# IBM/spark-s3-shuffle

Hardware: AMD Instinct MI355X
Metric: shuffle_block_compress_checksum_throughput (higher is better)
Workload: dtype u8; 1 GPU; terasort-10g-200p-lz4; direction=compress, codec=lz4, checksum=adler32, partitions_per_map_task=200, map_task_bytes=134217700, map_tasks_per_gpu=8, task_threads_per_gpu=4, map_tasks_per_library_call=2, inputs=resident in HBM

## Files before the change

### spark-s3-shuffle_amd/csrc/lz4_window_engine.inc

```

#if defined(S3S_ENGINE_NO_SPEC)
#undef S3S_ENGINE_SPEC
#elif !defined(S3S_ENGINE_SPEC)
#define S3S_ENGINE_SPEC 1
#endif

#if defined(S3S_ENGINE_NO_DEFER) || !defined(S3S_ENGINE_SPEC)
#undef S3S_ENGINE_DEFER
#elif !defined(S3S_ENGINE_DEFER)
#define S3S_ENGINE_DEFER 1
#endif

#ifdef S3S_LZ4_RING
#if !defined(S3S_ENGINE_SPEC) || !defined(S3S_ENGINE_DEFER) || defined(S3S_ENGINE_PW_DIRECT) || defined(S3S_ENGINE_DLOAD_20)
#error "S3S_LZ4_RING is built on the shipped block (speculative gather, deferred emission, 64-lane stream load)"
#endif
#define S3S_RING_SPAN "0xe80"
#define S3S_RING_BYTES 4096
#define S3S_RING_SPAN_N 0xe80
#define S3S_RING_AHEAD 316
#define S3S_RING_LANES 60
#if S3S_RING_SPAN_N - 1 + 64 + S3S_RING_AHEAD > S3S_RING_BYTES || 63 + 4 + 4 * (S3S_RING_LANES - 1) + 8 > S3S_RING_AHEAD
#error "S3S_RING_SPAN / S3S_RING_LANES no longer fit what the ring holds behind and ahead of a window"
#endif
#define S3S_RING_WRITE(OFF)                  \
  "v_add_u32_e32 v158, " OFF ", v158\n\t"                                                                  \
  "v_and_b32_e32 v158, 0xfff, v158\n\t"                                                                    \
  "ds_write_b32 v158, v154 offset:16384\n\t"
#define S3S_RING_FILL_ISSUE       \
  "v_lshl_add_u32 v150, v129, 4, s76\n\t"                                                                  \
  "v_add_u32_e32 v151, 0xfffff040, v150\n\t"                                                               \
  "v_add_u32_e32 v152, 0xfffff440, v150\n\t"                                                               \
  "v_add_u32_e32 v153, 0xfffff840, v150\n\t"                                                               \
// ... 48 lines not shown
  "s_and_saveexec_b64 s[84:85], s[82:83]\n\t"                                                              \
  "v_sub_u32_e32 v123, s97, v129\n\t"                                                                      \
  "v_sub_u32_e32 v124, s98, v129\n\t"                                                                      \
  "v_and_b32_e32 v123, 0xfff, v123\n\t"                                                                    \
  "v_and_b32_e32 v124, 0xfff, v124\n\t"                                                                    \
  "ds_read_u8 v127, v123 offset:16384\n\t"                                                                 \
  "ds_read_u8 v128, v124 offset:16384\n\t"                                                                 \
  "s_mov_b64 exec, s[84:85]\n\t"
#define S3S_RING_EXT(NB)                                                                                      \
  "s_cmpk_lt_u32 s98, " S3S_RING_SPAN "\n\t"                                                               \
  "s_cbranch_scc0 .Lw_extg" NB "_%=\n\t"                                                                   \
  S3S_RING_ISSUE                                                                                           \
  "s_and_b32 s97, s87, 0xc00000\n\t"                                                                       \
  "s_cbranch_scc1 .Lw_mfullr" NB "_%=\n\t"                                                                 \
  ".Lw_fwonlyr" NB "_%=:\n\t"                                                                              \
  S3S_RING_FIN                                                                                             \
  "v_xor_b32_e32 v123, v150, v151\n\t"                                                                     \
  "s_branch .Lw_fwc2" NB "_%=\n\t"                                                                        \
  ".Lw_mfullr" NB "_%=:\n\t"                                                                               \
  "s_bitcmp1_b32 s87, 23\n\t"                                                                              \
  "s_cbranch_scc1 .Lw_extbr" NB "_%=\n\t"                                                                  \
  "s_cmp_gt_i32 s92, 4\n\t"                                                                                \
  "s_cbranch_scc0 .Lw_fwonlyr" NB "_%=\n\t"                                                                \
  ".Lw_extbr" NB "_%=:\n\t"                                                                                \
  S3S_RING_BWD                                                                                             \
  S3S_RING_FIN                                                                                             \
  "v_cmp_ne_u32_e64 s[84:85], v127, v128\n\t"                                                              \
  "v_xor_b32_e32 v123, v150, v151\n\t"                                                                     \
  "s_branch .Lw_extbc2" NB "_%=\n\t"                                                                        \
    \
  ".Lw_mfullx" NB "_%=:\n\t"                                                                               \
  "s_bitcmp1_b32 s87, 23\n\t"                                                                              \
  "s_cbranch_scc1 .Lw_extbx" NB "_%=\n\t"                                                                  \
  "s_cmp_gt_i32 s92, 4\n\t"                                                                                \
  "s_cbranch_scc0 .Lw_exthw" NB "_%=\n\t"                                                                  \
  ".Lw_extbx" NB "_%=:\n\t"                                                                                \
  "s_sub_i32 s98, s89, s88\n\t"                                                                            \
  "s_cmpk_lt_u32 s98, " S3S_RING_SPAN "\n\t"                                                               \
  "s_cbranch_scc0 .Lw_extb" NB "_%=\n\t"                                                                   \
  S3S_RING_BWD                                                                                             \
  "s_waitcnt vmcnt(2) lgkmcnt(0)\n\t"                                                                      \
  "s_branch .Lw_extbc" NB "_%=\n\t"                                                                        \
  ".Lw_extg" NB "_%=:\n\t"
#define S3S_RING_EXTFULL(NB)                                                                                  \
  "s_cmpk_lt_u32 s98, " S3S_RING_SPAN "\n\t"                                                               \
  "s_cbranch_scc0 .Lw_extfg" NB "_%=\n\t"                                                                  \
  S3S_RING_ISSUE                                                                                           \
  "s_branch .Lw_extbr" NB "_%=\n\t"                                                                        \
  ".Lw_extfg" NB "_%=:\n\t"
#define S3S_RING_EXTBC(NB) ".Lw_extbc" NB "_%=:\n\t"
#define S3S_RING_EXTBC2(NB) ".Lw_extbc2" NB "_%=:\n\t"
#define S3S_RING_FWC2(NB) ".Lw_fwc2" NB "_%=:\n\t"
#define S3S_RING_EXTH_MFULL(NB) "s_cbranch_scc1 .Lw_mfullx" NB "_%=\n\t"
#define S3S_RING_EXTHW(NB) ".Lw_exthw" NB "_%=:\n\t"
#else
#define S3S_RING_WRITE(OFF)
#define S3S_RING_FILL_ISSUE
#define S3S_RING_FILL_WRITE
#define S3S_RING_EXT(NB)
#define S3S_RING_EXTFULL(NB)
#define S3S_RING_EXTBC(NB)
#define S3S_RING_EXTBC2(NB)
#define S3S_RING_FWC2(NB)
#define S3S_RING_EXTH_MFULL(NB) "s_cbranch_scc1 .Lw_mfull" NB "_%=\n\t"
#define S3S_RING_EXTHW(NB)
#endif

#ifdef S3S_ENGINE_ABL_NOSTORE
#define S3S_ENGINE_STORE ""
#else
#define S3S_ENGINE_STORE "global_store_byte v124, v122, %[outp]\n\t"
#endif

#ifdef S3S_ABL_CLAMP_FAR
#define S3S_ENGINE_STR_(x) #x
#define S3S_ENGINE_STR(x) S3S_ENGINE_STR_(x)
#define S3S_ENGINE_ABL_CLAMP "v_add_u32_e32 v152, -" S3S_ENGINE_STR(S3S_ABL_CLAMP_FAR) ", v148\n\tv_max_i32_e32 v150, v150, v152\n\t"
#else
#define S3S_ENGINE_ABL_CLAMP ""
#endif
#ifdef S3S_ABL_DUP_PW
#define S3S_ENGINE_ABL_DUP_PW "global_load_dwordx4 v[160:163], v148, %[inp] offset:124\n\t"
#else
// ... 244 lines not shown
  "ds_write_b16 v149, v148\n\t"                                                                            \
  "ds_read_u16 v128, v149\n\t"
#define S3S_SPEC_PASS2_AND_NEXT_GATHER(GN)                                                                    \
  "s_waitcnt lgkmcnt(0)\n\t"                                 \
  "v_cmp_ne_u32_e64 %[Dp], v128, v148\n\t"                                                                 \
  \
  "s_mov_b64 exec, -1\n\t"                                                                                 \
  "v_add_u32_e32 v150, -4, v159\n\t"                                                                       \
  "v_max_i32_e32 v150, 0, v150\n\t"                                                                        \
  "global_load_dwordx4 " GN ", v150, %[inp]" S3S_ENGINE_GATHER_POL "\n\t"                                    \
  "s_mov_b64 exec, %[Dp]\n\t"                                                                              \
  "ds_write_b16 v149, v148\n\t"                                                                            \
  "s_mov_b64 exec, s[74:75]\n\t"                                                                           \
  "ds_read_u16 v128, v149\n\t"  \
  S3S_ENGINE_RUN_INIT
#define S3S_SPEC_PASS2_DONE(FILL)                                                                             \
  "s_waitcnt lgkmcnt(0)\n\t"                                                                               \
  "v_cmp_ne_u32_e64 s[84:85], v128, v148\n\t"                                      \
  FILL                                                                                                     \
  "s_or_b64 %[Dp], %[Dp], s[84:85]\n\t"                                                                    \
  "s_andn2_b64 exec, s[74:75], s[84:85]\n\t"                                                               \
  "ds_write_b16 v149, %[cp]\n\t"                                                                           \
  "s_mov_b64 exec, -1\n\t"
#define S3S_ENGINE_FIXED(NB, Y0, Y1, Y2, Y3, Z0, Z1, Z2, Z3, G, G0, G1, G2, G3, GN)                            \
  ".Lw_winf" NB "_%=:\n\t"                                                                                 \
  S3S_SPEC_HEAD(Z0, Z1, Z2, Z3, "v_cmp_ne_u32_e64 vcc, %[cp], v159\n\t")                     \
  "v_mov_b32_e32 v150, 0x80000000\n\t"  \
  "v_cndmask_b32_e32 %[info], %[info], v150, vcc\n\t"                         \
  "v_cmp_ne_u32_e64 s[82:83], 0, %[info]\n\t"          \
  S3S_SPEC_PASS2_AND_NEXT_GATHER(GN)                                                                       \
  S3S_SPEC_PASS2_DONE("")                                                                                  \
  "s_or_b64 %[ED], s[82:83], %[Dp]\n\t"
#define S3S_SPEC_MISS_BODY(Z0, Z1, Z2, Z3, G, GN)                                                              \
  S3S_SPEC_HEAD(Z0, Z1, Z2, Z3, "")                                                                        \
  "v_cmp_gt_u32_e32 vcc, 4, %[cp]\n\t"           \
  "v_add_u32_e32 v150, -4, %[cp]\n\t"                                                                      \
  "v_max_i32_e32 v150, 0, v150\n\t"                                                                        \
  "global_load_dwordx4 " G ", v150, %[inp]" S3S_ENGINE_GATHER_POL "\n\t"                                     \
  "s_mov_b32 %[code], -1\n\t"                                                                              \
  S3S_SPEC_PASS2_AND_NEXT_GATHER(GN)                                                                       \
  S3S_SPEC_PASS2_DONE("")
#define S3S_ENGINE_FIXED_MISS(NB, X0, X1, X2, X3, Y0, Y1, Y2, Y3, Z0, Z1, Z2, Z3, G, G0, G1, G2, G3, GN)       \
  ".Lw_winm" NB "_%=:\n\t"                                                                                 \
  S3S_SPEC_MISS_BODY(Z0, Z1, Z2, Z3, G, GN)                                                                 \
  "s_waitcnt vmcnt(1)\n\t"                                                                                 \
  ".Lw_info" NB "_%=:\n\t"                                                                                 \
  S3S_ENGINE_INFO(Y0, Y1, Y2, Y3, G0, G1, G2, G3, "%[cp]", S3S_ENGINE_LIVE_AND)                             \
  "s_or_b64 %[ED], s[82:83], %[Dp]\n\t"                                                                    \
  "s_branch .Lw_top" NB "_%=\n\t"                                                                          \
  \
                        \
  ".Lw_fix" NB "_%=:\n\t"                                                                                  \
  "v_cmp_gt_i32_e32 vcc, 0, %[info]\n\t"                           \
  "s_add_i32 s97, s76, -64\n\t"                                                                            \
  "v_subrev_u32_e32 v150, s97, %[cp]\n\t"                                                                  \
  "v_cmp_gt_u32_e64 s[84:85], 64, v150\n\t"                                                                \
  "s_and_b64 s[84:85], s[84:85], vcc\n\t"                                                                  \
  "s_cmp_lt_u32 s76, 0x80\n\t" \
  "s_cselect_b64 s[84:85], 0, s[84:85]\n\t"                                                                \
  "s_bitcmp1_b64 s[84:85], s86\n\t"                                                                        \
  "s_cbranch_scc0 .Lw_regather" NB "_%=\n\t"                                                               \
  "s_andn2_b64 s[72:73], vcc, s[84:85]\n\t"                                          \
  "v_lshlrev_b32_e32 v152, 2, v150\n\t"                                                                    \
  "ds_bpermute_b32 v120, v152, " X0 "\n\t"                                                                 \
// ... 3 lines not shown
  "v_cmp_gt_u32_e32 vcc, 4, %[cp]\n\t"                                                                     \
  "s_mov_b32 %[code], -1\n\t"                                                                              \
  "s_waitcnt lgkmcnt(0)\n\t"                                                                               \
  "v_cndmask_b32_e64 " G0 ", " G0 ", v120, s[84:85]\n\t"                                                   \
  "v_cndmask_b32_e64 " G1 ", " G1 ", v121, s[84:85]\n\t"                                                   \
  "v_cndmask_b32_e64 " G2 ", " G2 ", v122, s[84:85]\n\t"                                                   \
  "v_cndmask_b32_e64 " G3 ", " G3 ", v123, s[84:85]\n\t"                                                   \
  S3S_ENGINE_INFO(Y0, Y1, Y2, Y3, G0, G1, G2, G3, "%[cp]", S3S_ENGINE_LIVE_AND)                             \
  "s_or_b64 %[ED], s[82:83], %[Dp]\n\t"                                                                    \
  "s_mov_b64 vcc, s[72:73]\n\t"                                                                            \
  "v_mov_b32_e32 v150, 0x80000000\n\t"                                                                     \
  "s_or_b64 %[ED], %[ED], s[72:73]\n\t"                                                                    \
  "v_cndmask_b32_e32 %[info], %[info], v150, vcc\n\t"                                                      \
  "s_branch .Lw_top" NB "_%=\n\t"                                                                          \
             \
  ".Lw_regather" NB "_%=:\n\t"                                                                             \
  "v_cmp_gt_u32_e32 vcc, 4, %[cp]\n\t"                                                                     \
  "v_add_u32_e32 v150, -4, %[cp]\n\t"                                                                      \
  "v_max_i32_e32 v150, 0, v150\n\t"                                                                        \
  "global_load_dwordx4 " G ", v150, %[inp]" S3S_ENGINE_GATHER_POL "\n\t"                                     \
  "s_mov_b32 %[code], -1\n\t"                                                                              \
  "s_waitcnt vmcnt(0)\n\t"                                                                                 \
  "s_branch .Lw_info" NB "_%=\n\t"                                                                         \
       \
  ".Lw_exth" NB "_%=:\n\t"                                                                                 \
  "s_and_b32 s97, s87, 0xc00000\n\t"                                                                       \
  S3S_RING_EXTH_MFULL(NB)                                                                                  \
  S3S_RING_EXTHW(NB)                                                                                       \
  "s_waitcnt vmcnt(2)\n\t"                                                                                 \
  "s_branch .Lw_fwcmp" NB "_%=\n\t"                                                                        \
  S3S_ENGINE_NVW(NB)
#define S3S_ENGINE_NEXT_TABLE_READ(Z1)                             \
  "v_mov_b32_e32 v149, v155\n\t"                                                                           \
  "ds_read_u16 %[cp], v149\n\t"
#define S3S_ENGINE_WIN_ENTRY(NB) "s_branch .Lw_winm" NB "_%=\n\t"
#define S3S_ENGINE_SPEC_ENTRY "s_mov_b32 %[code], -1\n\t"
#define S3S_ENGINE_SPEC_DUP(NB)                                                                               \
  "s_cmp_lt_i32 s87, 0\n\t"                                                                                \
  "s_cbranch_scc1 .Lw_fix" NB "_%=\n\t"
#define S3S_ENGINE_SPEC_X2(NB)                                                                                \
  "v_cmp_gt_i32_e32 vcc, 0, %[info]\n\t"                                                                   \
  "s_cmp_lg_u64 vcc, 0\n\t"                                                                                \
  "s_cbranch_scc1 .Lw_regather" NB "_%=\n\t"
#define S3S_ENGINE_SPEC_EXT(NB)                                                                               \
  "s_cmp_eq_u32 s86, %[code]\n\t"                                                                          \
  "s_mov_b32 %[code], -1\n\t"                                                                              \
  "s_cbranch_scc1 .Lw_exth" NB "_%=\n\t"
#define S3S_ENGINE_SPEC_EXTFULL(NB) "s_mov_b32 %[code], -1\n\t"
#define S3S_ENGINE_SPEC_FWCMP(NB) ".Lw_fwcmp" NB "_%=:\n\t"
#ifdef S3S_ENGINE_DEFER
#define S3S_ENGINE_SPEC_NOEV(NB)
#define S3S_ENGINE_NVW(NB)
#define S3S_ENGINE_WEND_VMCNT "s_waitcnt vmcnt(0)\n\t"
// ... 45 lines not shown
#ifndef S3S_ENGINE_SPEC
#define S3S_ENGINE_COMMIT(NB, Z0, Z1, Z2, Z3, N0, N1, N2, N3)                                                   \
  ".Lw_commit" NB "_%=:\n\t"                                                                                \
  "s_mov_b64 exec, %[K]\n\t"                                                                               \
  "ds_write_b16 v149, v148\n\t"                                                                            \
  "s_and_b64 s[82:83], %[K], %[Dp]\n\t"                                                                    \
  "s_bcnt1_i32_b64 s97, s[82:83]\n\t"                                                                      \
  "s_cmp_lt_u32 s97, 2\n\t"                                                                                \
  "s_cbranch_scc1 .Lw_cdone" NB "_%=\n\t"                                                                  \
  ".Lw_cloop" NB "_%=:\n\t"                                                                                 \
  "ds_read_u16 v151, v149\n\t"                                                                             \
  "s_waitcnt lgkmcnt(0)\n\t"                                                                               \
  "v_cmp_lt_u32_e64 s[82:83], v151, v148\n\t"                                                              \
  "s_cmp_eq_u64 s[82:83], 0\n\t"                                                                           \
  "s_cbranch_scc1 .Lw_cdone" NB "_%=\n\t"                                                                  \
  "s_mov_b64 exec, s[82:83]\n\t"                                                                           \
  "ds_write_b16 v149, v148\n\t"                                                                            \
  "s_mov_b64 exec, %[K]\n\t"                                                                               \
  "s_branch .Lw_cloop" NB "_%=\n\t"                                                                        \
  ".Lw_cdone" NB "_%=:\n\t"                                                                                 \
  "s_mov_b64 exec, -1\n\t"
#define S3S_ENGINE_CFIX(NB)
#define S3S_ENGINE_PERM_AT_END S3S_ENGINE_PW2_PERM
#else
#define S3S_ENGINE_COMMIT(NB, Z0, Z1, Z2, Z3, N0, N1, N2, N3)                                                   \
  ".Lw_commit" NB "_%=:\n\t"                                                                                \
  "s_mov_b64 exec, %[K]\n\t"                                                                               \
  "ds_write_b16 v149, v148\n\t"                                                                            \
  "ds_read_u16 v128, v149\n\t"                                                                             \
  "s_mov_b64 exec, -1\n\t"                                                                                 \
  S3S_ENGINE_SPEC_COMMIT(NB, Z0, Z1, Z2, Z3, N0, N1, N2, N3)                                                \
  "s_waitcnt lgkmcnt(0)\n\t"                                                                               \
  "s_mov_b64 exec, %[K]\n\t"                                                                               \
  "v_cmp_lt_u32_e64 s[82:83], v128, v148\n\t"                                                              \
  "s_mov_b64 exec, -1\n\t"                                                                                 \
  "v_mov_b32_e32 %[h], v156\n\t"                                                                           \
  S3S_ENGINE_PW2_PERM                                                                                      \
  "s_cmp_eq_u64 s[82:83], 0\n\t"                                                                           \
  "s_cbranch_scc0 .Lw_cfix" NB "_%=\n\t"                                                                   \
  ".Lw_cdone" NB "_%=:\n\t"
#define S3S_ENGINE_CFIX(NB)                                                                                   \
  ".Lw_cfix" NB "_%=:\n\t"                                                                                 \
  "s_mov_b64 exec, s[82:83]\n\t"                                                                           \
  "ds_write_b16 v149, v148\n\t"                                                                            \
  "s_mov_b64 exec, %[K]\n\t"                                                                               \
  "ds_read_u16 v128, v149\n\t"                                                                             \
  "s_waitcnt lgkmcnt(0)\n\t"                                                                               \
  "v_cmp_lt_u32_e64 s[82:83], v128, v148\n\t"                                                              \
  "s_mov_b64 exec, -1\n\t"                                                                                 \
  "s_cmp_eq_u64 s[82:83], 0\n\t"                                                                           \
  "s_cbranch_scc0 .Lw_cfix" NB "_%=\n\t"                                                                   \
  "s_branch .Lw_cdone" NB "_%=\n\t"
#define S3S_ENGINE_PERM_AT_END
// ... 240 lines not shown
  "s_mov_b64 exec, -1\n\t"
#define S3S_ENGINE_PEND_FAR(NB)                                                                               \
  "s_mul_i32 s98, s98, s79\n\t"                                                                            \
  "s_lshr_b32 s98, s98, 18\n\t"                                                                            \
  "s_and_b32 s98, s98, 0x3ffe\n\t"                                                                         \
  "v_mov_b32_e32 v150, s98\n\t"                                                                            \
  "v_mov_b32_e32 v151, %[pendq]\n\t"                                                                       \
  "ds_write_b16 v150, v151\n\t"                                                                            \
  "s_branch .Lw_nopend" NB "_%=\n\t"
#else
#define S3S_ENGINE_PEND_NEXT(NB, Z1)                                                                          \
  "s_add_i32 s97, s97, -64\n\t"                                                                            \
  "v_readlane_b32 s98, " Z1 ", s97\n\t"                                                                    \
  ".Lw_pendset" NB "_%=:\n\t"                                                                              \
  "s_mul_i32 s98, s98, s79\n\t"                                                                            \
  "s_lshr_b32 s98, s98, 18\n\t"                                                                            \
  "s_and_b32 s98, s98, 0x3ffe\n\t"                                                                         \
  "v_mov_b32_e32 v150, s98\n\t"                                                                            \
  "v_mov_b32_e32 v151, %[pendq]\n\t"                                                                       \
  "ds_write_b16 v150, v151\n\t"
#define S3S_ENGINE_PEND_FAR(NB) "s_branch .Lw_pendset" NB "_%=\n\t"
#endif

#define S3S_ENGINE_STEP(B, NB, NNB, TAIL, X, X0, X1, X2, X3, XLO, XHI, Y, Y0, Y1, Y2, Y3, YLO, YHI, Z, Z0, Z1, Z2, \
                        Z3, ZLO, ZHI, G, G0, G1, G2, G3, GN, N0, N1, N2, N3)                                  \
             \
  ".Lw_disp" B "_%=:\n\t"                                                                                   \
  "v_add_u32_e32 v148, s76, v129\n\t"                                                                      \
  "s_sub_i32 s97, s76, %[pk]\n\t"                                                                          \
  "s_cmp_eq_u32 s97, 64\n\t"                                                                               \
  "s_cbranch_scc0 .Lw_dispx" B "_%=\n\t"                                                                   \
  "v_mov_b32_e32 %[vp], " X1 "\n\t"                                                                        \
  "s_mov_b32 %[pk], s76\n\t"                                                                               \
  S3S_ENGINE_PW2_COMMON(X)                                                                                 \
  S3S_ENGINE_ABL_DUP_PW                                                                                    \
                   \
  \
  S3S_ENGINE_FIXED(NB, Y0, Y1, Y2, Y3, Z0, Z1, Z2, Z3, G, G0, G1, G2, G3, GN)                                    \
                  \
  ".Lw_top" NB "_%=:\n\t"                                                                                  \
  "s_and_b64 s[82:83], s[80:81], %[ED]\n\t"                                                                \
  "s_cbranch_scc0 .Lw_noev" NB "_%=\n\t"                                                                   \
  S3S_ENGINE_TOP(NB)                                                                                       \
  "s_cmp_gt_i32 s92, 4\n\t"                                                                                \
  "s_cselect_b32 s97, 0x480000, s77\n\t"                                                                   \
  "s_and_b32 s97, s97, s87\n\t"                                                                            \
  "s_cbranch_scc0 .Lw_len" NB "_%=\n\t"                                                                    \
  \
  ".Lw_ext" NB "_%=:\n\t"                                                                                  \
  S3S_ENGINE_SPEC_EXT(NB)                                                                                  \
  "s_add_i32 s97, s89, 4\n\t"                                                                              \
  "v_lshl_add_u32 v125, v129, 2, s97\n\t"                                                                  \
  "s_sub_i32 s98, s89, s88\n\t"                                                                            \
  "v_subrev_u32_e32 v126, s98, v125\n\t"                                                                   \
  S3S_RING_EXT(NB)                                                                                         \
  "global_load_dword v130, v125, %[inp]\n\t"                                                               \
  S3S_ENGINE_ABL_DUP_IPSIDE                                                                                \
  "global_load_dword v131, v126, %[inp]\n\t"                                                               \
  "s_and_b32 s97, s87, 0xc00000\n\t"                                                                       \
  "s_cbranch_scc1 .Lw_mfull" NB "_%=\n\t"                                                                  \
  ".Lw_fwonly" NB "_%=:\n\t"                                                                               \
  "s_waitcnt vmcnt(0)\n\t"                                                                                 \
  S3S_ENGINE_SPEC_FWCMP(NB)                                                                                \
  "v_cmp_ne_u32_e64 s[82:83], v130, v131\n\t"                                                              \
  "v_xor_b32_e32 v123, v130, v131\n\t"                                                                     \
  S3S_RING_FWC2(NB)                                                                                        \
  "s_cmp_eq_u64 s[82:83], 0\n\t"                                                                           \
  "s_cbranch_scc1 .Lw_x2" NB "_%=\n\t"                                                                     \
  "s_ff1_i32_b64 s98, s[82:83]\n\t"                                                                        \
  "v_readlane_b32 s90, v123, s98\n\t"                                                                      \
  "s_ff1_i32_b32 s90, s90\n\t"                                                                             \
  "s_lshr_b32 s90, s90, 3\n\t"                                                                             \
  "s_lshl2_add_u32 s90, s98, s90\n\t"                                                                      \
                                                                                \
  ".Lw_len" NB "_%=:\n\t"                                                                                   \
  "s_sub_i32 s93, s92, s91\n\t"                                                                            \
  "s_add_i32 s94, s91, s90\n\t"                                                                            \
  S3S_ENGINE_SEQ_BYTES                                                                                     \
  "s_add_i32 s97, s93, 0xff\n\t"                                                                           \
  "s_max_i32 s97, s97, s94\n\t"                                                                            \
  "s_cmpk_gt_i32 s97, 0x10d\n\t"                                                                           \
  "s_cbranch_scc1 .Lw_x2" NB "_%=\n\t"                                                                     \
  S3S_ENGINE_EMIT(Y1)                                                                                        \
  S3S_ENGINE_OP_ADVANCE                                                                                    \
  "s_sub_i32 %[rs], %[anchor], s76\n\t"                                                                    \
  "s_add_i32 s98, %[rs], -2\n\t"                                                                           \
  "s_cmp_lt_i32 %[rs], 64\n\t"                                                                             \
  "s_cbranch_scc0 .Lw_leave" NB "_%=\n\t"                                                                  \
  "s_bitset1_b64 %[K], s98\n\t"                                                                            \
  "s_lshl_b64 s[80:81], -1, %[rs]\n\t"                                                                     \
  "s_branch .Lw_top" NB "_%=\n\t"                                                                          \
  \
  ".Lw_leave" NB "_%=:\n\t"                                                                                \
  "s_add_i32 s99, %[anchor], -2\n\t"                                                                       \
  "s_lshl_b64 s[82:83], 1, s98\n\t"                                                                        \
  "s_cmp_lt_i32 s98, 64\n\t"                                                                               \
  "s_cselect_b64 s[82:83], s[82:83], 0\n\t"                                                                \
  "s_cselect_b32 %[pendq], %[pendq], s99\n\t"                                                              \
  "s_or_b64 %[K], %[K], s[82:83]\n\t"                                                                      \
  "s_mov_b32 %[base], %[anchor]\n\t"                                                                       \
  "s_mov_b32 %[t0], 0\n\t"                                                                                 \
  "s_branch .Lw_commit" NB "_%=\n\t"                                                                       \
                                                           \
  ".Lw_mfull" NB "_%=:\n\t"                                                                                \
  "s_bitcmp1_b32 s87, 23\n\t"                                                                              \
  "s_cbranch_scc1 .Lw_extb" NB "_%=\n\t"                                                                   \
  "s_cmp_gt_i32 s92, 4\n\t"                                                                                \
  "s_cbranch_scc0 .Lw_fwonly" NB "_%=\n\t"                                                                 \
  "s_branch .Lw_extb" NB "_%=\n\t"                                                                         \
  ".Lw_extfull" NB "_%=:\n\t"                                                                              \
  S3S_ENGINE_SPEC_EXTFULL(NB)                                                                              \
  "s_add_i32 s97, s89, 4\n\t"                                                                              \
  "v_lshl_add_u32 v125, v129, 2, s97\n\t"                                                                  \
  "s_sub_i32 s98, s89, s88\n\t"                                                                            \
  "v_subrev_u32_e32 v126, s98, v125\n\t"                                                                   \
  S3S_RING_EXTFULL(NB)                                                                                     \
  "global_load_dword v130, v125, %[inp]\n\t"                                                               \
  S3S_ENGINE_ABL_DUP_IPSIDE                                                                                \
  "global_load_dword v131, v126, %[inp]\n\t"                                                               \
  ".Lw_extb" NB "_%=:\n\t"                                                                                 \
  "s_min_i32 s99, s92, s88\n\t"                                                                            \
  "v_mov_b32_e32 v127, 0\n\t"                                                                              \
  "v_mov_b32_e32 v128, 1\n\t"                                                                              \
  "v_cmp_gt_i32_e64 s[82:83], s99, v129\n\t"                                                               \
  "s_add_i32 s97, s89, -1\n\t"                                                                             \
  "s_add_i32 s98, s88, -1\n\t"                                                                             \
  "s_and_saveexec_b64 s[84:85], s[82:83]\n\t"                                                              \
  "v_sub_u32_e32 v123, s97, v129\n\t"                                                                      \
  "v_sub_u32_e32 v124, s98, v129\n\t"                                                                      \
  "global_load_ubyte v127, v123, %[inp]\n\t"                                                               \
  "global_load_ubyte v128, v124, %[inp]\n\t"                                                               \
  "s_mov_b64 exec, s[84:85]\n\t"                                                                           \
  "s_waitcnt vmcnt(0)\n\t"                                                                                 \
  S3S_RING_EXTBC(NB)                                                                                       \
  "v_cmp_ne_u32_e64 s[82:83], v130, v131\n\t"                                                              \
  "v_cmp_ne_u32_e64 s[84:85], v127, v128\n\t"                                                              \
  "v_xor_b32_e32 v123, v130, v131\n\t"                                                                     \
  S3S_RING_EXTBC2(NB)                                                                                      \
  "s_ff1_i32_b64 s97, s[84:85]\n\t"                                                                        \
  "s_min_u32 s97, s97, 63\n\t"                                                                             \
  "s_cmp_eq_u32 s97, 63\n\t"                                                                               \
  "s_cbranch_scc1 .Lw_x2" NB "_%=\n\t"                                                                     \
  "s_cmp_eq_u64 s[82:83], 0\n\t"                                                                           \
  "s_cbranch_scc1 .Lw_x2" NB "_%=\n\t"                                                                     \
  "s_ff1_i32_b64 s98, s[82:83]\n\t"                                                                        \
  "v_readlane_b32 s90, v123, s98\n\t"                                                                      \
  "s_ff1_i32_b32 s90, s90\n\t"                                                                             \
  "s_lshr_b32 s90, s90, 3\n\t"                                                                             \
  "s_lshl2_add_u32 s90, s98, s90\n\t"                                                                      \
  ".Lw_got" NB "_%=:\n\t"                                                                                   \
  "s_mov_b32 s91, s97\n\t"                                                                                 \
  "s_branch .Lw_len" NB "_%=\n\t"                                                                          \
  \
            \
  ".Lw_dup" NB "_%=:\n\t"                                                                                  \
  S3S_ENGINE_SPEC_DUP(NB)                                                                                  \
  "v_readlane_b32 s88, %[h], s86\n\t"                                                                      \
  "s_or_b64 s[84:85], s[80:81], %[K]\n\t"                                                                  \
  "s_nop 0\n\t"                                                                                            \
  "v_cmp_eq_u32_e64 s[82:83], s88, %[h]\n\t"                                                               \
// ... 1 lines not shown
  "s_lshl_b64 s[84:85], -1, s86\n\t"                                                                       \
  "s_andn2_b64 s[82:83], s[82:83], s[84:85]\n\t"                                                           \
  "s_cbranch_scc0 .Lw_dupnone" NB "_%=\n\t"                                                                \
  "s_flbit_i32_b64 s97, s[82:83]\n\t"                                                                      \
  "s_sub_i32 s97, 63, s97\n\t"                                                                             \
  "v_readlane_b32 s98, " Y1 ", s97\n\t"                                                                    \
  "v_readlane_b32 s99, " Y1 ", s86\n\t"                                                                    \
  "s_cmp_eq_u32 s98, s99\n\t"                                                                              \
  "s_cbranch_scc0 .Lw_clear" NB "_%=\n\t"                                                                  \
  "s_add_i32 s88, s76, s97\n\t"                                                                            \
  "s_add_i32 s89, s76, s86\n\t"                                                                            \
  "s_sub_i32 s92, s89, %[anchor]\n\t"                                                                      \
  "s_branch .Lw_extfull" NB "_%=\n\t"                                                                          \
  ".Lw_dupnone" NB "_%=:\n\t"                                                                              \
  "s_bitcmp0_b32 s87, 30\n\t"                                                                              \
  "s_cbranch_scc1 .Lw_clear" NB "_%=\n\t"                                                                  \
  "s_and_b32 s88, s87, 0xffff\n\t"                                                                         \
  "s_branch .Lw_dkok" NB "_%=\n\t"                                                                         \
  ".Lw_clear" NB "_%=:\n\t"                                                                                \
  "s_lshl_b64 s[84:85], 1, s86\n\t"                                                                        \
  "s_andn2_b64 %[ED], %[ED], s[84:85]\n\t"                                                                 \
  "s_branch .Lw_top" NB "_%=\n\t"                                                                          \
  S3S_ENGINE_FIXED_MISS(NB, X0, X1, X2, X3, Y0, Y1, Y2, Y3, Z0, Z1, Z2, Z3, G, G0, G1, G2, G3, GN)               \
  S3S_ENGINE_CFIX(NB)                                                                                      \
  S3S_ENGINE_FLUSH_STUB(NB)                                                                                \
  ".Lw_out0" NB "_%=:\n\t"                                                                                 \
  "s_mov_b32 %[code], 0\n\t"                                                                               \
  "s_branch .Lw_out" NB "_%=\n\t"                                                                          \
  ".Lw_x2" NB "_%=:\n\t"                                                                                    \
  S3S_ENGINE_SPEC_X2(NB)                                                                                   \
  "s_cmp_lg_u64 %[K], 0\n\t"                                                                               \
  "s_cselect_b64 %[valid], -1, %[valid]\n\t"                                                               \
  "s_mov_b32 %[code], 2\n\t"                                                                               \
                      \
  ".Lw_out" NB "_%=:\n\t"                                                                                   \
  "s_waitcnt vmcnt(0) lgkmcnt(0)\n\t"                                                                      \
  S3S_ENGINE_FLUSH_AT_EXIT(NB)                                                                             \
  S3S_ENGINE_PW2_EXIT(X0, X1, X2, X3)                                                                      \
  "s_add_i32 %[kp], %[pk], -64\n\t"                                                                        \
  "v_mov_b64 %[p0l], " YLO "\n\t"                                                                          \
  "v_mov_b64 %[p0h], " YHI "\n\t"                                                                          \
  "v_mov_b64 %[p1l], " ZLO "\n\t"                                                                          \
  "v_mov_b64 %[p1h], " ZHI "\n\t"                                                                          \
  "v_mov_b64 %[p2l], " XLO "\n\t"                                                                          \
  "v_mov_b64 %[p2h], " XHI "\n\t"                                                                          \
  "s_branch .Lw_end_%=\n\t"                                                                                \
                                                   \
  ".Lw_pendb" NB "_%=:\n\t"                                                                                \
  S3S_ENGINE_PENDB_REGS(NB, X1)                                                                            \
  ".Lw_pendc" NB "_%=:\n\t"                                                                                \
  "v_mov_b32_e32 v151, %[pendq]\n\t"                                                                       \
  "global_load_dword v150, v151, %[inp]\n\t"                                                               \
  "s_waitcnt vmcnt(0)\n\t"                                                                                 \
// ... 18 lines not shown
  "s_branch .Lw_win" NNB "_%=\n\t"                                                                         \
  ".Lw_dispf" B "_%=:\n\t"                                                                                  \
  "s_mov_b32 %[pk], s76\n\t"                                                                               \
  "global_load_dwordx4 " X ", v148, %[inp] offset:-4\n\t"                                                  \
  S3S_ENGINE_DISP_FAR(Y, Z)                                                                                \
  "s_branch .Lw_win" B "_%=\n\t"                                                                           \
  ".Lw_same" B "_%=:\n\t"                                                                                  \
  S3S_ENGINE_DISP_SAME(Y, Z)                                                                               \
  "s_branch .Lw_win" B "_%=\n\t"                                                                           \
                           \
  ".Lw_noev" NB "_%=:\n\t"                                                                                  \
  "s_sub_i32 s97, s78, %[t0]\n\t"                                                                          \
  "s_add_i32 s97, s97, 66\n\t"                                                                             \
  "s_min_i32 s97, s97, 64\n\t"                                                                             \
  "s_cmp_lg_u64 %[K], 0\n\t"                                                                               \
  "s_cselect_b32 s97, 64, s97\n\t"                                                                         \
  "s_cselect_b32 s98, 0, %[t0]\n\t"                                                                        \
  S3S_ENGINE_SPEC_NOEV(NB)                                                                                 \
  "s_or_b64 %[K], %[K], s[80:81]\n\t"                                                                      \
  "s_add_i32 %[base], s76, s97\n\t"                                                                        \
  "s_add_i32 s98, s98, s97\n\t"                                                                            \
  "s_sub_i32 %[t0], s98, %[rs]\n\t"                                                                        \
  \
                                      \
  S3S_ENGINE_COMMIT(NB, Z0, Z1, Z2, Z3, N0, N1, N2, N3)                                                    \
  \
  "s_cmp_lt_i32 %[pendq], 0\n\t"                                                                           \
  "s_cbranch_scc1 .Lw_nopend" NB "_%=\n\t"                                                                 \
  "s_sub_i32 s97, %[pendq], s76\n\t"                                                                       \
  "s_cmpk_lt_i32 s97, 0x80\n\t"                                                                            \
  "s_cbranch_scc0 .Lw_pendb" NB "_%=\n\t"                                                                  \
  S3S_ENGINE_PEND_NEXT(NB, Z1)                                                                             \
  ".Lw_nopend" NB "_%=:\n\t"                                                                                \
  \
  S3S_ENGINE_NEXT_TABLE_READ(Z1)                                                                           \
  S3S_ENGINE_PERM_AT_END                                                                                      \
  S3S_ENGINE_COND_RING(".Lw_out0" NB "_%=")                                                                \
  S3S_ENGINE_FLUSH_AT_WINDOW_END(NB)                                                                       \
  TAIL

#define S3S_RA "v[132:135]", "v132", "v133", "v134", "v135", "v[132:133]", "v[134:135]"
#define S3S_RB "v[136:139]", "v136", "v137", "v138", "v139", "v[136:137]", "v[138:139]"
#define S3S_RC "v[140:143]", "v140", "v141", "v142", "v143", "v[140:141]", "v[142:143]"
#define S3S_ENGINE_STEP_(B, NB, NNB, TAIL, ...) S3S_ENGINE_STEP(B, NB, NNB, TAIL, __VA_ARGS__)
#define S3S_G0 "v[144:147]", "v144", "v145", "v146", "v147"
#ifdef S3S_ENGINE_SPEC
// ... 43 lines not shown
```

Baseline: 118.9 GB/s.

## Speculatively pre-insert hash-table entries ahead of window and relayout extension blocks

Adds a DUP_AHEAD path that writes the next position into the LZ4 hash table early and reads it back to detect lane duplicates, then rolls back at commit or window exit when the speculation is wrong. This aims to overlap the table update with the gather load instead of serialising it at commit. It also adds a LAYOUT option that moves the match-extension and leave blocks out of line or merges them into fallthrough to cut branches on the hot path. Both are on by default, at the cost of extra LDS traffic and rollback logic.

```diff
diff --git a/spark-s3-shuffle_amd/csrc/lz4_window_engine.inc b/spark-s3-shuffle_amd/csrc/lz4_window_engine.inc
--- a/spark-s3-shuffle_amd/csrc/lz4_window_engine.inc
+++ b/spark-s3-shuffle_amd/csrc/lz4_window_engine.inc
@@ -9,6 +9,18 @@
 #undef S3S_ENGINE_DEFER
 #elif !defined(S3S_ENGINE_DEFER)
 #define S3S_ENGINE_DEFER 1
+#endif
+
+#if defined(S3S_ENGINE_NO_DUP_AHEAD) || !defined(S3S_ENGINE_DEFER)
+#undef S3S_ENGINE_DUP_AHEAD
+#elif !defined(S3S_ENGINE_DUP_AHEAD)
+#define S3S_ENGINE_DUP_AHEAD 1
+#endif
+
+#if defined(S3S_ENGINE_LAYOUT_R6)
+#undef S3S_ENGINE_LAYOUT
+#elif !defined(S3S_ENGINE_LAYOUT)
+#define S3S_ENGINE_LAYOUT 1
 #endif
 
 #ifdef S3S_LZ4_RING
@@ -103,12 +115,7 @@
   "s_cbranch_scc1 .Lw_extbr" NB "_%=\n\t"                                                                  \
   "s_cmp_gt_i32 s92, 4\n\t"                                                                                \
   "s_cbranch_scc0 .Lw_fwonlyr" NB "_%=\n\t"                                                                \
-  ".Lw_extbr" NB "_%=:\n\t"                                                                                \
-  S3S_RING_BWD                                                                                             \
-  S3S_RING_FIN                                                                                             \
-  "v_cmp_ne_u32_e64 s[84:85], v127, v128\n\t"                                                              \
-  "v_xor_b32_e32 v123, v150, v151\n\t"                                                                     \
-  "s_branch .Lw_extbc2" NB "_%=\n\t"                                                                        \
+  S3S_RING_EXTBR_HERE(NB)                                                                                  \
     \
   ".Lw_mfullx" NB "_%=:\n\t"                                                                               \
   "s_bitcmp1_b32 s87, 23\n\t"                                                                              \
@@ -123,12 +130,34 @@
   "s_waitcnt vmcnt(2) lgkmcnt(0)\n\t"                                                                      \
   "s_branch .Lw_extbc" NB "_%=\n\t"                                                                        \
   ".Lw_extg" NB "_%=:\n\t"
+#ifdef S3S_ENGINE_LAYOUT
+#define S3S_RING_EXTBR_HERE(NB) "s_branch .Lw_extbr" NB "_%=\n\t"
+#define S3S_RING_EXTFULL(NB)                                                                                  \
+  "s_cmpk_lt_u32 s98, " S3S_RING_SPAN "\n\t"                                                               \
+  "s_cbranch_scc0 .Lw_extfg" NB "_%=\n\t"                                                                  \
+  S3S_RING_ISSUE                                                                                           \
+  ".Lw_extbr" NB "_%=:\n\t"                                                                                \
+  S3S_RING_BWD                                                                                             \
+  S3S_RING_FIN                                                                                             \
+  "v_cmp_ne_u32_e64 s[84:85], v127, v128\n\t"                                                              \
+  "v_xor_b32_e32 v123, v150, v151\n\t"
+#define S3S_RING_EXTFG(NB) ".Lw_extfg" NB "_%=:\n\t"
+#else
+#define S3S_RING_EXTBR_HERE(NB)                                                                               \
+  ".Lw_extbr" NB "_%=:\n\t"                                                                                \
+  S3S_RING_BWD                                                                                             \
+  S3S_RING_FIN                                                                                             \
+  "v_cmp_ne_u32_e64 s[84:85], v127, v128\n\t"                                                              \
+  "v_xor_b32_e32 v123, v150, v151\n\t"                                                                     \
+  "s_branch .Lw_extbc2" NB "_%=\n\t"
 #define S3S_RING_EXTFULL(NB)                                                                                  \
   "s_cmpk_lt_u32 s98, " S3S_RING_SPAN "\n\t"                                                               \
   "s_cbranch_scc0 .Lw_extfg" NB "_%=\n\t"                                                                  \
   S3S_RING_ISSUE                                                                                           \
   "s_branch .Lw_extbr" NB "_%=\n\t"                                                                        \
   ".Lw_extfg" NB "_%=:\n\t"
+#define S3S_RING_EXTFG(NB)
+#endif
 #define S3S_RING_EXTBC(NB) ".Lw_extbc" NB "_%=:\n\t"
 #define S3S_RING_EXTBC2(NB) ".Lw_extbc2" NB "_%=:\n\t"
 #define S3S_RING_FWC2(NB) ".Lw_fwc2" NB "_%=:\n\t"
@@ -140,6 +169,7 @@
 #define S3S_RING_FILL_WRITE
 #define S3S_RING_EXT(NB)
 #define S3S_RING_EXTFULL(NB)
+#define S3S_RING_EXTFG(NB)
 #define S3S_RING_EXTBC(NB)
 #define S3S_RING_EXTBC2(NB)
 #define S3S_RING_FWC2(NB)
@@ -430,6 +460,53 @@
   "s_andn2_b64 exec, s[74:75], s[84:85]\n\t"                                                               \
   "ds_write_b16 v149, %[cp]\n\t"                                                                           \
   "s_mov_b64 exec, -1\n\t"
+#ifdef S3S_ENGINE_DUP_AHEAD
+#define S3S_DUPA_PASS1                                                                                        \
+  "v_add_u32_e32 v117, 64, v148\n\t"                                                                       \
+  "ds_write_b16 v155, v117\n\t"                                                                            \
+  "ds_read_u16 v116, v155\n\t"
+#define S3S_DUPA_PASS2                                                                                        \
+  "s_mov_b64 exec, s[84:85]\n\t"                                                                           \
+  "ds_write_b16 v155, v117\n\t"                                                                            \
+  "s_mov_b64 exec, -1\n\t"                                                                                 \
+  "ds_read_u16 v115, v155\n\t"
+#define S3S_DUPA_ROLLBACK                                                             \
+  "v_cmpx_eq_u32_e32 vcc, v115, v117\n\t"                                                             \
+  "ds_write_b16 v155, v159\n\t"
+#define S3S_ENGINE_FIXED(NB, Y0, Y1, Y2, Y3, Z0, Z1, Z2, Z3, G, G0, G1, G2, G3, GN)                            \
+  ".Lw_winf" NB "_%=:\n\t"                                                                                 \
+  "s_sub_i32 s78, %[base], s76\n\t"                                                                        \
+  "v_cmp_le_u32_e64 s[74:75], s78, v129\n\t"                                                               \
+  "s_waitcnt lgkmcnt(0)\n\t"                \
+  S3S_ENGINE_PW1_ALIGN(Z0, Z1, Z2, Z3)                                                                      \
+  "v_mul_lo_u32 v155, " Z1 ", s79\n\t"                                                                     \
+  "v_cmp_ne_u32_e64 vcc, %[cp], v159\n\t"                                                 \
+  "v_lshrrev_b32_e32 v156, 19, v155\n\t"                                                                   \
+  "v_lshlrev_b32_e32 v155, 1, v156\n\t"                                                                    \
+  "ds_read_u16 v159, v155\n\t" \
+  S3S_DUPA_PASS1                                                                                           \
+  "s_mov_b64 exec, s[74:75]\n\t"                                                                           \
+  "v_mov_b32_e32 v150, 0x80000000\n\t"  \
+  "v_cndmask_b32_e32 %[info], %[info], v150, vcc\n\t"                         \
+  "v_cmp_ne_u32_e64 s[82:83], 0, %[info]\n\t"          \
+  "s_mov_b64 exec, -1\n\t"                                                                                 \
+  "s_and_b64 %[Dp], %[Dp], s[74:75]\n\t"                                                                   \
+  S3S_ENGINE_RUN_INIT                                                                                      \
+  "s_waitcnt lgkmcnt(0)\n\t"                                        \
+  "v_cmp_ne_u32_e64 s[84:85], v116, v117\n\t"                                                              \
+  \
+  "v_add_u32_e32 v150, -4, v159\n\t"                                                                       \
+  "v_max_i32_e32 v150, 0, v150\n\t"                                                                        \
+  "global_load_dwordx4 " GN ", v150, %[inp]" S3S_ENGINE_GATHER_POL "\n\t"                                    \
+  "s_or_b64 %[ED], s[82:83], %[Dp]\n\t"                                                                    \
+  S3S_DUPA_PASS2
+#define S3S_DUPA_MISS  \
+  S3S_DUPA_PASS1                                                                                           \
+  "s_waitcnt lgkmcnt(0)\n\t"                                                                               \
+  "v_cmp_ne_u32_e64 s[84:85], v116, v117\n\t"                                                              \
+  S3S_DUPA_PASS2
+#else
+#define S3S_DUPA_MISS
 #define S3S_ENGINE_FIXED(NB, Y0, Y1, Y2, Y3, Z0, Z1, Z2, Z3, G, G0, G1, G2, G3, GN)                            \
   ".Lw_winf" NB "_%=:\n\t"                                                                                 \
   S3S_SPEC_HEAD(Z0, Z1, Z2, Z3, "v_cmp_ne_u32_e64 vcc, %[cp], v159\n\t")                     \
@@ -439,6 +516,7 @@
   S3S_SPEC_PASS2_AND_NEXT_GATHER(GN)                                                                       \
   S3S_SPEC_PASS2_DONE("")                                                                                  \
   "s_or_b64 %[ED], s[82:83], %[Dp]\n\t"
+#endif
 #define S3S_SPEC_MISS_BODY(Z0, Z1, Z2, Z3, G, GN)                                                              \
   S3S_SPEC_HEAD(Z0, Z1, Z2, Z3, "")                                                                        \
   "v_cmp_gt_u32_e32 vcc, 4, %[cp]\n\t"           \
@@ -447,7 +525,8 @@
   "global_load_dwordx4 " G ", v150, %[inp]" S3S_ENGINE_GATHER_POL "\n\t"                                     \
   "s_mov_b32 %[code], -1\n\t"                                                                              \
   S3S_SPEC_PASS2_AND_NEXT_GATHER(GN)                                                                       \
-  S3S_SPEC_PASS2_DONE("")
+  S3S_SPEC_PASS2_DONE("")                                                                                  \
+  S3S_DUPA_MISS
 #define S3S_ENGINE_FIXED_MISS(NB, X0, X1, X2, X3, Y0, Y1, Y2, Y3, Z0, Z1, Z2, Z3, G, G0, G1, G2, G3, GN)       \
   ".Lw_winm" NB "_%=:\n\t"                                                                                 \
   S3S_SPEC_MISS_BODY(Z0, Z1, Z2, Z3, G, GN)                                                                 \
@@ -497,13 +576,6 @@
   "s_mov_b32 %[code], -1\n\t"                                                                              \
   "s_waitcnt vmcnt(0)\n\t"                                                                                 \
   "s_branch .Lw_info" NB "_%=\n\t"                                                                         \
-       \
-  ".Lw_exth" NB "_%=:\n\t"                                                                                 \
-  "s_and_b32 s97, s87, 0xc00000\n\t"                                                                       \
-  S3S_RING_EXTH_MFULL(NB)                                                                                  \
-  S3S_RING_EXTHW(NB)                                                                                       \
-  "s_waitcnt vmcnt(2)\n\t"                                                                                 \
-  "s_branch .Lw_fwcmp" NB "_%=\n\t"                                                                        \
   S3S_ENGINE_NVW(NB)
 #define S3S_ENGINE_NEXT_TABLE_READ(Z1)                             \
   "v_mov_b32_e32 v149, v155\n\t"                                                                           \
@@ -595,13 +667,31 @@
   "s_mov_b64 exec, -1\n\t"
 #define S3S_ENGINE_CFIX(NB)
 #define S3S_ENGINE_PERM_AT_END S3S_ENGINE_PW2_PERM
-#else
+#define S3S_DUPA_X2
+#else
+#ifdef S3S_ENGINE_DUP_AHEAD
+#define S3S_DUPA_COMMIT_HEAD                                                                                  \
+  "s_waitcnt lgkmcnt(0)\n\t"                                                                               \
+  "v_cmp_ne_u32_e64 s[82:83], v116, v117\n\t"           \
+  S3S_DUPA_ROLLBACK
+#define S3S_DUPA_COMMIT_DP "s_orn2_b64 %[Dp], s[82:83], vcc\n\t"
+#define S3S_DUPA_X2                                                                                           \
+  "s_waitcnt lgkmcnt(0)\n\t"                                                                               \
+  S3S_DUPA_ROLLBACK                                                                                        \
+  "s_mov_b64 exec, -1\n\t"
+#else
+#define S3S_DUPA_COMMIT_HEAD
+#define S3S_DUPA_COMMIT_DP
+#define S3S_DUPA_X2
+#endif
 #define S3S_ENGINE_COMMIT(NB, Z0, Z1, Z2, Z3, N0, N1, N2, N3)                                                   \
   ".Lw_commit" NB "_%=:\n\t"                                                                                \
+  S3S_DUPA_COMMIT_HEAD                                                                                     \
   "s_mov_b64 exec, %[K]\n\t"                                                                               \
   "ds_write_b16 v149, v148\n\t"                                                                            \
   "ds_read_u16 v128, v149\n\t"                                                                             \
   "s_mov_b64 exec, -1\n\t"                                                                                 \
+  S3S_DUPA_COMMIT_DP                                                                                       \
   S3S_ENGINE_SPEC_COMMIT(NB, Z0, Z1, Z2, Z3, N0, N1, N2, N3)                                                \
   "s_waitcnt lgkmcnt(0)\n\t"                                                                               \
   "s_mov_b64 exec, %[K]\n\t"                                                                               \
@@ -888,6 +978,104 @@
 #define S3S_ENGINE_PEND_FAR(NB) "s_branch .Lw_pendset" NB "_%=\n\t"
 #endif
 
+#define S3S_ENGINE_EXT_ADDR                                                                                   \
+  "s_add_i32 s97, s89, 4\n\t"                                                                              \
+  "v_lshl_add_u32 v125, v129, 2, s97\n\t"                                                                  \
+  "s_sub_i32 s98, s89, s88\n\t"                                                                            \
+  "v_subrev_u32_e32 v126, s98, v125\n\t"
+#define S3S_ENGINE_EXT_LOADS                                                                                  \
+  "global_load_dword v130, v125, %[inp]\n\t"                                                               \
+  S3S_ENGINE_ABL_DUP_IPSIDE                                                                                \
+  "global_load_dword v131, v126, %[inp]\n\t"
+#define S3S_ENGINE_EXT_ONDEMAND(NB)                                                                           \
+  S3S_ENGINE_EXT_ADDR                                                                                      \
+  S3S_RING_EXT(NB)                                                                                         \
+  S3S_ENGINE_EXT_LOADS                                                                                     \
+  "s_and_b32 s97, s87, 0xc00000\n\t"                                                                       \
+  "s_cbranch_scc1 .Lw_mfull" NB "_%=\n\t"                                                                  \
+  ".Lw_fwonly" NB "_%=:\n\t"                                                                               \
+  "s_waitcnt vmcnt(0)\n\t"
+#define S3S_ENGINE_EXT_EARLY(NB)                                                                              \
+  ".Lw_exth" NB "_%=:\n\t"                                                                                 \
+  "s_and_b32 s97, s87, 0xc00000\n\t"                                                                       \
+  S3S_RING_EXTH_MFULL(NB)                                                                                  \
+  S3S_RING_EXTHW(NB)                                                                                       \
+  "s_waitcnt vmcnt(2)\n\t"
+#if !defined(S3S_ENGINE_SPEC)
+#define S3S_ENGINE_EXT_INLINE(NB) S3S_ENGINE_EXT_ONDEMAND(NB)
+#define S3S_ENGINE_EXT_OUTLINE(NB)
+#elif !defined(S3S_ENGINE_LAYOUT)
+#define S3S_ENGINE_EXT_INLINE(NB)                                                                             \
+  S3S_ENGINE_SPEC_EXT(NB)                                                                                  \
+  S3S_ENGINE_EXT_ONDEMAND(NB)
+#define S3S_ENGINE_EXT_OUTLINE(NB)                                                                            \
+  S3S_ENGINE_EXT_EARLY(NB)                                                                                 \
+  "s_branch .Lw_fwcmp" NB "_%=\n\t"
+#else
+#define S3S_ENGINE_EXT_INLINE(NB)                                                                             \
+  "s_cmp_eq_u32 s86, %[code]\n\t"                                                                          \
+  "s_mov_b32 %[code], -1\n\t"                                                                              \
+  "s_cbranch_scc0 .Lw_extd" NB "_%=\n\t"                                                                   \
+  S3S_ENGINE_EXT_EARLY(NB)
+#define S3S_ENGINE_EXT_OUTLINE(NB)                                                                            \
+  ".Lw_extd" NB "_%=:\n\t"                                                                                 \
+  S3S_ENGINE_EXT_ONDEMAND(NB)                                                                              \
+  "s_branch .Lw_fwcmp" NB "_%=\n\t"
+#endif
+#define S3S_ENGINE_EXTB(NB)                                                                                   \
+  ".Lw_extb" NB "_%=:\n\t"                                                                                 \
+  "s_min_i32 s99, s92, s88\n\t"                                                                            \
+  "v_mov_b32_e32 v127, 0\n\t"                                                                              \
+  "v_mov_b32_e32 v128, 1\n\t"                                                                              \
+  "v_cmp_gt_i32_e64 s[82:83], s99, v129\n\t"                                                               \
+  "s_add_i32 s97, s89, -1\n\t"                                                                             \
+  "s_add_i32 s98, s88, -1\n\t"                                                                             \
+  "s_and_saveexec_b64 s[84:85], s[82:83]\n\t"                                                              \
+  "v_sub_u32_e32 v123, s97, v129\n\t"                                                                      \
+  "v_sub_u32_e32 v124, s98, v129\n\t"                                                                      \
+  "global_load_ubyte v127, v123, %[inp]\n\t"                                                               \
+  "global_load_ubyte v128, v124, %[inp]\n\t"                                                               \
+  "s_mov_b64 exec, s[84:85]\n\t"                                                                           \
+  "s_waitcnt vmcnt(0)\n\t"                                                                                 \
+  S3S_RING_EXTBC(NB)                                                                                       \
+  "v_cmp_ne_u32_e64 s[82:83], v130, v131\n\t"                                                              \
+  "v_cmp_ne_u32_e64 s[84:85], v127, v128\n\t"                                                              \
+  "v_xor_b32_e32 v123, v130, v131\n\t"
+#if defined(S3S_LZ4_RING) && defined(S3S_ENGINE_LAYOUT)
+#define S3S_ENGINE_EXTB_INLINE(NB)
+#define S3S_ENGINE_EXTB_OUTLINE(NB)                                                                           \
+  S3S_RING_EXTFG(NB)                                                                                       \
+  S3S_ENGINE_EXT_LOADS                                                                                     \
+  S3S_ENGINE_EXTB(NB)                                                                                      \
+  "s_branch .Lw_extbc2" NB "_%=\n\t"
+#else
+#define S3S_ENGINE_EXTB_INLINE(NB)                                                                            \
+  S3S_ENGINE_EXT_LOADS                                                                                     \
+  S3S_ENGINE_EXTB(NB)
+#define S3S_ENGINE_EXTB_OUTLINE(NB)
+#endif
+#define S3S_ENGINE_LEAVE(NB)                                                                                  \
+  ".Lw_leave" NB "_%=:\n\t"                                                                                \
+  "s_add_i32 s99, %[anchor], -2\n\t"                                                                       \
+  "s_lshl_b64 s[82:83], 1, s98\n\t"                                                                        \
+  "s_cmp_lt_i32 s98, 64\n\t"                                                                               \
+  "s_cselect_b64 s[82:83], s[82:83], 0\n\t"                                                                \
+  "s_cselect_b32 %[pendq], %[pendq], s99\n\t"                                                              \
+  "s_or_b64 %[K], %[K], s[82:83]\n\t"                                                                      \
+  "s_mov_b32 %[base], %[anchor]\n\t"                                                                       \
+  "s_mov_b32 %[t0], 0\n\t"
+#ifdef S3S_ENGINE_LAYOUT
+#define S3S_ENGINE_LEAVE_R6(NB)
+#define S3S_ENGINE_LEAVE_AT_COMMIT(NB)                                                                        \
+  "s_branch .Lw_commit" NB "_%=\n\t"                                                                       \
+  S3S_ENGINE_LEAVE(NB)
+#else
+#define S3S_ENGINE_LEAVE_R6(NB)                                                                               \
+  S3S_ENGINE_LEAVE(NB)                                                                                     \
+  "s_branch .Lw_commit" NB "_%=\n\t"
+#define S3S_ENGINE_LEAVE_AT_COMMIT(NB)
+#endif
+
 #define S3S_ENGINE_STEP(B, NB, NNB, TAIL, X, X0, X1, X2, X3, XLO, XHI, Y, Y0, Y1, Y2, Y3, YLO, YHI, Z, Z0, Z1, Z2, \
                         Z3, ZLO, ZHI, G, G0, G1, G2, G3, GN, N0, N1, N2, N3)                                  \
              \
@@ -914,19 +1102,7 @@
   "s_cbranch_scc0 .Lw_len" NB "_%=\n\t"                                                                    \
   \
   ".Lw_ext" NB "_%=:\n\t"                                                                                  \
-  S3S_ENGINE_SPEC_EXT(NB)                                                                                  \
-  "s_add_i32 s97, s89, 4\n\t"                                                                              \
-  "v_lshl_add_u32 v125, v129, 2, s97\n\t"                                                                  \
-  "s_sub_i32 s98, s89, s88\n\t"                                                                            \
-  "v_subrev_u32_e32 v126, s98, v125\n\t"                                                                   \
-  S3S_RING_EXT(NB)                                                                                         \
-  "global_load_dword v130, v125, %[inp]\n\t"                                                               \
-  S3S_ENGINE_ABL_DUP_IPSIDE                                                                                \
-  "global_load_dword v131, v126, %[inp]\n\t"                                                               \
-  "s_and_b32 s97, s87, 0xc00000\n\t"                                                                       \
-  "s_cbranch_scc1 .Lw_mfull" NB "_%=\n\t"                                                                  \
-  ".Lw_fwonly" NB "_%=:\n\t"                                                                               \
-  "s_waitcnt vmcnt(0)\n\t"                                                                                 \
+  S3S_ENGINE_EXT_INLINE(NB)                                                                                \
   S3S_ENGINE_SPEC_FWCMP(NB)                                                                                \
   "v_cmp_ne_u32_e64 s[82:83], v130, v131\n\t"                                                              \
   "v_xor_b32_e32 v123, v130, v131\n\t"                                                                     \
@@ -956,17 +1132,7 @@
   "s_bitset1_b64 %[K], s98\n\t"                                                                            \
   "s_lshl_b64 s[80:81], -1, %[rs]\n\t"                                                                     \
   "s_branch .Lw_top" NB "_%=\n\t"                                                                          \
-  \
-  ".Lw_leave" NB "_%=:\n\t"                                                                                \
-  "s_add_i32 s99, %[anchor], -2\n\t"                                                                       \
-  "s_lshl_b64 s[82:83], 1, s98\n\t"                                                                        \
-  "s_cmp_lt_i32 s98, 64\n\t"                                                                               \
-  "s_cselect_b64 s[82:83], s[82:83], 0\n\t"                                                                \
-  "s_cselect_b32 %[pendq], %[pendq], s99\n\t"                                                              \
-  "s_or_b64 %[K], %[K], s[82:83]\n\t"                                                                      \
-  "s_mov_b32 %[base], %[anchor]\n\t"                                                                       \
-  "s_mov_b32 %[t0], 0\n\t"                                                                                 \
-  "s_branch .Lw_commit" NB "_%=\n\t"                                                                       \
+  S3S_ENGINE_LEAVE_R6(NB)                                                                                  \
                                                            \
   ".Lw_mfull" NB "_%=:\n\t"                                                                                \
   "s_bitcmp1_b32 s87, 23\n\t"                                                                              \
@@ -976,32 +1142,9 @@
   "s_branch .Lw_extb" NB "_%=\n\t"                                                                         \
   ".Lw_extfull" NB "_%=:\n\t"                                                                              \
   S3S_ENGINE_SPEC_EXTFULL(NB)                                                                              \
-  "s_add_i32 s97, s89, 4\n\t"                                                                              \
-  "v_lshl_add_u32 v125, v129, 2, s97\n\t"                                                                  \
-  "s_sub_i32 s98, s89, s88\n\t"                                                                            \
-  "v_subrev_u32_e32 v126, s98, v125\n\t"                                                                   \
+  S3S_ENGINE_EXT_ADDR                                                                                      \
   S3S_RING_EXTFULL(NB)                                                                                     \
-  "global_load_dword v130, v125, %[inp]\n\t"                                                               \
-  S3S_ENGINE_ABL_DUP_IPSIDE                                                                                \
-  "global_load_dword v131, v126, %[inp]\n\t"                                                               \
-  ".Lw_extb" NB "_%=:\n\t"                                                                                 \
-  "s_min_i32 s99, s92, s88\n\t"                                                                            \
-  "v_mov_b32_e32 v127, 0\n\t"                                                                              \
-  "v_mov_b32_e32 v128, 1\n\t"                                                                              \
-  "v_cmp_gt_i32_e64 s[82:83], s99, v129\n\t"                                                               \
-  "s_add_i32 s97, s89, -1\n\t"                                                                             \
-  "s_add_i32 s98, s88, -1\n\t"                                                                             \
-  "s_and_saveexec_b64 s[84:85], s[82:83]\n\t"                                                              \
-  "v_sub_u32_e32 v123, s97, v129\n\t"                                                                      \
-  "v_sub_u32_e32 v124, s98, v129\n\t"                                                                      \
-  "global_load_ubyte v127, v123, %[inp]\n\t"                                                               \
-  "global_load_ubyte v128, v124, %[inp]\n\t"                                                               \
-  "s_mov_b64 exec, s[84:85]\n\t"                                                                           \
-  "s_waitcnt vmcnt(0)\n\t"                                                                                 \
-  S3S_RING_EXTBC(NB)                                                                                       \
-  "v_cmp_ne_u32_e64 s[82:83], v130, v131\n\t"                                                              \
-  "v_cmp_ne_u32_e64 s[84:85], v127, v128\n\t"                                                              \
-  "v_xor_b32_e32 v123, v130, v131\n\t"                                                                     \
+  S3S_ENGINE_EXTB_INLINE(NB)                                                                               \
   S3S_RING_EXTBC2(NB)                                                                                      \
   "s_ff1_i32_b64 s97, s[84:85]\n\t"                                                                        \
   "s_min_u32 s97, s97, 63\n\t"                                                                             \
@@ -1049,6 +1192,8 @@
   "s_andn2_b64 %[ED], %[ED], s[84:85]\n\t"                                                                 \
   "s_branch .Lw_top" NB "_%=\n\t"                                                                          \
   S3S_ENGINE_FIXED_MISS(NB, X0, X1, X2, X3, Y0, Y1, Y2, Y3, Z0, Z1, Z2, Z3, G, G0, G1, G2, G3, GN)               \
+  S3S_ENGINE_EXT_OUTLINE(NB)                                                                               \
+  S3S_ENGINE_EXTB_OUTLINE(NB)                                                                              \
   S3S_ENGINE_CFIX(NB)                                                                                      \
   S3S_ENGINE_FLUSH_STUB(NB)                                                                                \
   ".Lw_out0" NB "_%=:\n\t"                                                                                 \
@@ -1056,6 +1201,7 @@
   "s_branch .Lw_out" NB "_%=\n\t"                                                                          \
   ".Lw_x2" NB "_%=:\n\t"                                                                                    \
   S3S_ENGINE_SPEC_X2(NB)                                                                                   \
+  S3S_DUPA_X2                                                                                              \
   "s_cmp_lg_u64 %[K], 0\n\t"                                                                               \
   "s_cselect_b64 %[valid], -1, %[valid]\n\t"                                                               \
   "s_mov_b32 %[code], 2\n\t"                                                                               \
@@ -1120,6 +1266,7 @@
   "s_add_i32 s98, s98, s97\n\t"                                                                            \
   "s_sub_i32 %[t0], s98, %[rs]\n\t"                                                                        \
   \
+  S3S_ENGINE_LEAVE_AT_COMMIT(NB)                                                                           \
                                       \
   S3S_ENGINE_COMMIT(NB, Z0, Z1, Z2, Z3, N0, N1, N2, N3)                                                    \
   \
```

Result: faster. 120.9 GB/s (median of 6 runs) (+1.6%).
